# karapostK/hassaku

Measured on AMD Instinct MI355X. Metric: BPR triplets/sec, higher is better.
Workload: dtype f32

## Files before the change

### hassaku_amd/_lib.py

```python
import ctypes
import os
from ctypes import POINTER, c_char_p, c_double, c_int, c_int32, c_int64, c_uint64, c_void_p

_HERE = os.path.dirname(os.path.abspath(__file__))
LIB_PATH = os.environ.get('HSK_LIB_PATH') or os.path.join(_HERE, 'libhassaku_hip.so')

_lib = None


class HskBprmfState(ctypes.Structure):
    _fields_ = [
        ('user_emb', c_void_p), ('item_emb', c_void_p), ('item_bias', c_void_p),
        ('user_bias', c_void_p), ('global_bias', c_void_p),
        ('m_user_emb', c_void_p), ('v_user_emb', c_void_p),
        ('m_item_emb', c_void_p), ('v_item_emb', c_void_p),
        ('m_item_bias', c_void_p), ('v_item_bias', c_void_p),
        ('m_user_bias', c_void_p), ('v_user_bias', c_void_p),
        ('m_global_bias', c_void_p), ('v_global_bias', c_void_p),
        ('n_users', c_int64), ('n_items', c_int64), ('dim', c_int64),
        ('lr', c_double), ('beta1', c_double), ('beta2', c_double), ('eps', c_double), ('wd', c_double),
        ('step', c_int64),
        ('csr_indptr', c_void_p), ('csr_indices', c_void_p),
        ('coo_user', c_void_p), ('coo_item', c_void_p),
        ('nnz', c_int64),
        ('seed', c_uint64),
        ('workspace', c_void_p), ('workspace_bytes', c_int64),
        ('max_batch', c_int64), ('max_cols', c_int64),
        ('lazy_users', c_int32), ('timing_mask', c_int32),
        ('timing', c_void_p), ('aux', c_void_p),
        ('timing_every', c_int32), ('loss_kind', c_int32),
        ('opt_kind', c_int32), ('lazy_items', c_int32),
        ('ssm_log_adjust', c_double),
        ('alias_prob', c_void_p), ('alias_idx', c_void_p),
        ('graph_chunk', c_int32), ('catchup_apart', c_int32),
        ('loss_out', c_void_p), ('status', c_void_p),
        ('flush_every', c_int32), ('ws_sharded', c_int32),
        ('frozen_hyper', c_double * 5), ('frozen_opt', c_int32), ('frozen_valid', c_int32),
        ('timing_now', c_int32), ('reserved3', c_int32),
    ]


class HskBprmfShard(ctypes.Structure):
    _fields_ = [
        ('base', HskBprmfState),
        ('world', c_int32), ('rank', c_int32),
        ('n_users_global', c_int64), ('n_items_global', c_int64),
        ('item_lo', c_int64), ('capacity', c_int64), ('entry_cap', c_int64),
        ('shard_ws', c_void_p), ('shard_ws_bytes', c_int64),
        ('rows_send', c_void_p), ('rows_all', c_void_p),
        ('dU_all', c_void_p), ('grads_mine', c_void_p),
        ('s0', c_void_p), ('gsum', c_void_p),
        ('ssm_send', c_void_p), ('ssm_all', c_void_p),
        ('cur_batch', c_int64), ('cur_cols', c_int64),
        ('cur_set', c_int32), ('phase', c_int32),
    ]


SIGNATURES = {
    'hsk_version': (c_int, []),
    'hsk_last_error': (c_char_p, []),
    'hsk_device_info': (c_int, [POINTER(c_int32), POINTER(c_int32), c_char_p, c_int32]),
    'hsk_mf_scores': (c_int, [c_void_p] * 5 + [c_int64] * 3 + [c_void_p, c_void_p, c_int64, c_int64,
                                                              c_void_p, c_void_p, c_void_p]),
    'hsk_bpr_loss_grad': (c_int, [c_void_p, c_int64, c_int64, c_void_p, c_void_p, c_void_p, c_void_p]),
    'hsk_rec_loss_grad': (c_int, [c_int32, c_void_p, c_int64, c_int64, c_double, c_void_p, c_void_p, c_void_p, c_void_p]),
    'hsk_mf_backward': (c_int, [c_void_p, c_void_p, c_int64, c_int64, c_int64, c_void_p, c_void_p, c_int64,
                                c_int64, c_void_p] + [c_void_p] * 5 + [c_void_p, c_void_p]),
    'hsk_embedding_gather': (c_int, [c_void_p, c_int64, c_int64, c_void_p, c_int64, c_void_p, c_void_p, c_void_p]),
    'hsk_embedding_backward_ws_bytes': (c_int64, [c_int64, c_int64]),
    'hsk_embedding_backward': (c_int, [c_void_p, c_void_p, c_int64, c_int64, c_int64, c_void_p, c_void_p, c_int64,
                                       c_void_p, c_void_p]),
    'hsk_sparse_rows_sum': (c_int, [c_void_p, c_int64, c_int64, c_void_p, c_void_p, c_int64, c_void_p, c_int64,
                                    c_void_p, c_void_p, c_void_p]),
    'hsk_sparse_rows_offsets': (c_int, [c_void_p, c_int64, c_void_p, c_int64, c_void_p, c_void_p, c_void_p]),
    'hsk_sparse_rows_sum_backward_ws_bytes': (c_int64, [c_int64, c_int64]),
    'hsk_sparse_rows_sum_backward': (c_int, [c_void_p, c_void_p, c_void_p, c_int64, c_int64, c_void_p, c_int64,
                                             c_void_p, c_int64, c_int64, c_void_p, c_void_p, c_int64, c_void_p,
                                             c_void_p]),
    'hsk_adamw_dense': (c_int, [c_void_p] * 4 + [c_int64] + [c_double] * 5 + [c_int64, c_void_p]),
    'hsk_opt_dense': (c_int, [c_int] + [c_void_p] * 4 + [c_int64] + [c_double] * 5 + [c_int64, c_void_p]),
    'hsk_sample_negatives_uniform': (c_int, [c_void_p, c_void_p, c_int64, c_int64, c_void_p, c_int64, c_int64,
                                             c_uint64, c_uint64, c_void_p, c_void_p, c_void_p]),
    'hsk_sample_negatives_alias': (c_int, [c_void_p, c_void_p, c_int64, c_int64, c_void_p, c_void_p, c_void_p, c_int64,
                                           c_int64, c_uint64, c_uint64, c_void_p, c_void_p, c_void_p]),
    'hsk_bprmf_workspace_bytes': (c_int64, [c_int64] * 5),
    'hsk_bprmf_flush_cadence': (c_int32, [POINTER(HskBprmfState), c_int32, c_int64]),
    'hsk_shard_base_workspace_bytes': (c_int64, [c_int64] * 5),
    'hsk_synth_degrees': (c_int, [c_int64, c_int32, c_int32, c_uint64, c_void_p, c_void_p]),
    'hsk_synth_fill': (c_int, [c_int64, c_int64, c_int32, c_int32, c_uint64, c_void_p, c_void_p, c_void_p, c_void_p]),
    'hsk_bprmf_init_workspace': (c_int, [POINTER(HskBprmfState), c_void_p]),
    'hsk_bprmf_train_step': (c_int, [POINTER(HskBprmfState), c_void_p, c_void_p, c_int64, c_int64, c_void_p]),
    'hsk_bprmf_train_step_sampled': (c_int, [POINTER(HskBprmfState), c_void_p, c_int64, c_int64, c_int64,
                                             c_void_p]),
    'hsk_bprmf_train_steps': (c_int, [POINTER(HskBprmfState), c_void_p, c_int64, c_int64, c_int64, c_int64,
                                      c_void_p]),
    'hsk_bprmf_last_sort': (c_int, [POINTER(HskBprmfState), c_int64, c_void_p, c_void_p, c_void_p]),
    'hsk_key_sort_plan': (c_int, [c_int64, c_int64, c_int, POINTER(c_int64)]),
    'hsk_key_sort_ws_bytes': (c_int64, [c_int64, c_int64, c_int]),
    'hsk_key_sort': (c_int, [c_void_p, c_int64, c_int64, c_void_p, c_void_p, c_void_p, c_void_p, c_void_p, c_void_p,
                             c_int64, c_void_p, c_void_p]),
    'hsk_bprmf_graph_replays': (c_int64, [POINTER(HskBprmfState)]),
    'hsk_bprmf_batch_columns': (c_int64, [POINTER(HskBprmfState), c_int64, c_int64]),
    'hsk_eval_set_arith': (None, [c_int]),
    'hsk_timing_create': (c_void_p, []),
    'hsk_timing_destroy': (None, [c_void_p]),
    'hsk_timing_collect': (c_int, [c_void_p, POINTER(c_double), POINTER(c_int64)]),
    'hsk_aux_create': (c_void_p, []),
    'hsk_aux_destroy': (None, [c_void_p]),
    'hsk_bprmf_hint_next': (c_int, [POINTER(HskBprmfState), c_void_p, c_int64, c_int64, c_int64]),
    'hsk_bprmf_hint_after_run': (c_int, [POINTER(HskBprmfState), c_void_p, c_int64, c_int64, c_int64]),
    'hsk_bprmf_hint_after_run_n': (c_int, [POINTER(HskBprmfState), c_void_p, c_int64, c_int64, c_int64, c_int64]),
    'hsk_bprmf_pipelined_steps': (c_int64, [POINTER(HskBprmfState)]),
    'hsk_bprmf_set_pipeline': (None, [c_int]),
    'hsk_shard_workspace_bytes': (c_int64, [c_int64] * 4),
    'hsk_shard_init': (c_int, [POINTER(HskBprmfShard), c_void_p]),
    'hsk_shard_prepare': (c_int, [POINTER(HskBprmfShard), c_void_p, c_int64, c_int64, c_int64, c_int32, c_void_p]),
    'hsk_shard_discard': (c_int, [POINTER(HskBprmfShard), c_int32, c_void_p]),
    'hsk_shard_pack': (c_int, [POINTER(HskBprmfShard), c_int64, c_int64, c_int32, c_void_p]),
    'hsk_shard_pos_scores': (c_int, [POINTER(HskBprmfShard), c_void_p]),
    'hsk_shard_forward': (c_int, [POINTER(HskBprmfShard), c_void_p]),
    'hsk_shard_pos_fix': (c_int, [POINTER(HskBprmfShard), c_void_p]),
# ... 105 lines not shown
```

### hassaku_amd/csrc/hsk_fused.hip

```cpp
#include <hip/hip_ext.h>
#include "hsk_sampler.h"
#include "hsk_sort.h"
#include "hsk_step_kernels.h"
#include "hsk_item_sliced.h"
#include "hsk_fwd_small.h"
#include "hsk_fwd_part.h"
#include <stdlib.h>

#include <algorithm>
#include <utility>
#include <vector>

#ifndef HSK_FWD_R
#define HSK_FWD_R 4
#endif
#ifndef HSK_FWD_PART_R
#define HSK_FWD_PART_R 3
#endif
#define HSK_ADAM_TAB_LEN 65536
#define HSK_FLUSH_NEVER (1 << 30)

#define HSK_PART_MAX 8
#define HSK_GROUP_MAX 8
static int hsk_group_rule(int64_t n_items, int64_t dim, int64_t batch, int64_t n_cols) {
// ... 530 lines not shown
  return hsk_flush_cadence(st, table, (double)touched_rows);
}

static int hsk_launch_flush(hsk_bprmf_state* st, const hsk_ws& w, hipStream_t stream, int which = 3,
                            const int* g_poison = nullptr) {
  const int U = (int)st->n_users, D = (int)st->dim;
  if (st->step == 0) return HSK_OK;
  const hsk_adamw_consts c = hsk_make_adamw_consts(st->lr, st->beta1, st->beta2, st->eps, st->wd, st->step, st->opt_kind);
#define HSK_FLUSH(VV, GEN)                                                                                       \
  k_user_flush<VV, GEN><<<(unsigned)U, 256, 0, stream>>>(st->user_emb, st->m_user_emb, st->v_user_emb, st->user_bias, \
                                                         st->m_user_bias, st->v_user_bias, w.last_step, U, D,         \
                                                         (int)st->step, c, w.adam_tab, HSK_ADAM_TAB_LEN, g_poison)
  const bool gen = st->opt_kind != HSK_OPT_ADAMW;
  static const int wave_on = getenv("HSK_FLUSH_WAVE") ? atoi(getenv("HSK_FLUSH_WAVE")) : 1;
  const bool wave = wave_on && D <= 64 * 8 * ((D % 4 == 0) ? 4 : (D % 2 == 0) ? 2 : 1);
  auto wave_sweep = [&](float* P, float* M, float* V_, float* Pb, float* Mb, float* Vb, int* last, int n_rows) {
    return hsk_dispatch_dim(D, [&](auto v_, auto n_, auto f_) {
      constexpr int V = decltype(v_)::value, NCH = decltype(n_)::value;
      constexpr bool FULL = decltype(f_)::value;
      const unsigned grid = (unsigned)((n_rows + 3) / 4);
      if (gen)
        k_row_flush_wave<V, NCH, FULL, true><<<grid, 256, 0, stream>>>(P, M, V_, Pb, Mb, Vb, last, n_rows, D, (int)st->step, c,
                                                                     w.adam_tab, HSK_ADAM_TAB_LEN, g_poison);
      else
        k_row_flush_wave<V, NCH, FULL, false><<<grid, 256, 0, stream>>>(P, M, V_, Pb, Mb, Vb, last, n_rows, D, (int)st->step, c,
                                                                      w.adam_tab, HSK_ADAM_TAB_LEN, g_poison);
      return HSK_OK;
    });
  };
  if (wave) {
    if (st->lazy_users && (which & 1)) {
      const int rc = wave_sweep(st->user_emb, st->m_user_emb, st->v_user_emb, st->user_bias, st->m_user_bias, st->v_user_bias,
                                w.last_step, U);
      if (rc != HSK_OK) return rc;
    }
    if (st->lazy_items && (which & 2)) {
      const int rc = wave_sweep(st->item_emb, st->m_item_emb, st->v_item_emb, st->item_bias, st->m_item_bias, st->v_item_bias,
                                w.last_step_i, (int)st->n_items);
      if (rc != HSK_OK) return rc;
    }
    HSK_LAUNCH_CHECK();
    return HSK_OK;
  }
  if (st->lazy_users && (which & 1)) {
    if (D % 2 == 0) {
      if (gen) HSK_FLUSH(2, true); else HSK_FLUSH(2, false);
    } else {
      if (gen) HSK_FLUSH(1, true); else HSK_FLUSH(1, false);
    }
  }
#undef HSK_FLUSH
  if (st->lazy_items && (which & 2)) {
    const int I = (int)st->n_items;
    if (gen)
      k_user_flush<2, true><<<(unsigned)I, 256, 0, stream>>>(st->item_emb, st->m_item_emb, st->v_item_emb, st->item_bias,
                                                            st->m_item_bias, st->v_item_bias, w.last_step_i, I, D,
                                                            (int)st->step, c, w.adam_tab, HSK_ADAM_TAB_LEN, g_poison);
    else
      k_user_flush<2, false><<<(unsigned)I, 256, 0, stream>>>(st->item_emb, st->m_item_emb, st->v_item_emb, st->item_bias,
                                                             st->m_item_bias, st->v_item_bias, w.last_step_i, I, D,
                                                             (int)st->step, c, w.adam_tab, HSK_ADAM_TAB_LEN, g_poison);
  }
  HSK_LAUNCH_CHECK();
  return HSK_OK;
}

static int hsk_periodic_flush(hsk_bprmf_state* st, const hsk_ws& w, hipStream_t stream, int64_t step_before,
                              double user_rows, double entries, const int* g_poison = nullptr) {
  int which = 0;
  if (st->lazy_users) {
    const int64_t F = hsk_flush_cadence(st, 0, user_rows);
    if (st->step / F != step_before / F) which |= 1;
  }
  if (st->lazy_items) {
    const int64_t F = hsk_flush_cadence(st, 1, hsk_touched_rows((double)st->n_items, entries));
    if (st->step / F != step_before / F) which |= 2;
  }
  if (!which) return HSK_OK;
  int rc = HSK_OK;
  HSK_STAGE(HSK_STAGE_USER, rc = hsk_launch_flush(st, w, stream, which, g_poison));
  return rc;
}

template <int V, int NCH, bool FULL, int R, bool APPLY>
static void hsk_launch_item_pass(const hsk_bprmf_state* st, const hsk_ws& w, const float* Urows, const int* urow_index,
                                 int K, const hsk_adamw_consts& c, float* gI_out, float* gIb_out, hipStream_t stream,
                                 int64_t n_entries = 0, const hsk_user_lazy_args* ua = nullptr,
                                 const hsk_ahead_args* aa = nullptr, int n_part = 1, const int* g_ovf = nullptr,
                                 const int* g_poison = nullptr, const hsk_ride_item* ri = nullptr) {
  const bool part = n_part > 1;
  const int I = (int)st->n_items, D = (int)st->dim;
  if (D % 2 != 0) {
    k_item_update<V, NCH, FULL, R, APPLY><<<(unsigned)hsk_ceil_div(I, 4), 256, 0, stream>>>(
        Urows, st->item_emb, st->item_bias, st->m_item_emb, st->v_item_emb, st->m_item_bias, st->v_item_bias,
        urow_index, w.g_s, w.perm, w.offsets, I, K, D, c, gI_out, gIb_out, g_ovf, g_poison);
    return;
  }
  constexpr int VSC = (V == 4) ? 4 : 2;
  const int ipw = 1;
  const int vs = VSC;
  const int n_sl = (int)hsk_ceil_div(D, 64 * vs);
  static const int rows_on = getenv("HSK_ITEM_ROWS") ? atoi(getenv("HSK_ITEM_ROWS")) : 1;
  static const int rows_lazy = getenv("HSK_ITEM_ROWS_LAZY") ? atoi(getenv("HSK_ITEM_ROWS_LAZY")) : 1;
  const bool whole_rows = APPLY && ua && rows_on && (n_entries <= 64 * 1024 || (rows_lazy && st->lazy_items)) && !part;
  const int n_slices_pad = whole_rows ? 0 : (n_sl < 8 && 8 % n_sl == 0) ? n_sl : (int)hsk_align_up(n_sl, 8);
  const bool lazy = APPLY && st->lazy_items;
  const int64_t n_list = lazy ? std::min<int64_t>(I, n_entries) : I;
  const unsigned groups = (unsigned)hsk_align_up(hsk_ceil_div(n_list, 4 * ipw), 8);
  const hsk_item_args ia = {Urows, st->item_emb, st->item_bias, st->m_item_emb, st->v_item_emb, st->m_item_bias,
                            st->v_item_bias, urow_index, w.g_s, w.perm, w.offsets, I, K, D, n_slices_pad, ipw, c,
                            gI_out, gIb_out, w.touched, w.n_touched, w.last_step_i, (int)st->step, w.pend,
                            ua ? ua->desc : nullptr, ua ? ua->rel : 0, w.adam_tab, HSK_ADAM_TAB_LEN, n_part};
  const bool gen = APPLY && st->opt_kind != HSK_OPT_ADAMW;
  const unsigned nblk = groups * (whole_rows ? 1 : n_slices_pad);
  if (APPLY && ua) {
    const int dense = ua->n_users > 0;
    const int nub = (int)hsk_align_up(hsk_ceil_div(dense ? ua->n_users : ua->B, 4) + 1, 8);
    const hsk_ahead_args ahead = aa ? *aa : hsk_ahead_args{};
    const int item_oct = (int)(nblk / 8);
    int n_ahead_oct = ahead.coo_user ? (int)hsk_ceil_div(hsk_ceil_div(ahead.n, 4), 8) : 0;
    n_ahead_oct = std::min(n_ahead_oct, item_oct);
    const int stride = n_ahead_oct ? item_oct / n_ahead_oct : 0;
    const int nab_big = ahead.coo_user ? (int)hsk_align_up(hsk_ceil_div(ahead.n, 4), 8) : 0;

#define HSK_ITEM_USER(VS, GEN, LZ)                                                                             \
  do {                                                                                                         \
    if (whole_rows)                                                                                            \
      k_item_user_small<V, NCH, FULL, GEN, LZ><<<nblk + (unsigned)(nub + 8 * n_ahead_oct), 256, 0, stream>>>(    \
          ia, *ua, nub, dense, ahead, n_ahead_oct, stride);                                                    \
    else if (part) {                                                                                           \
      if constexpr (V == 4 && FULL && !LZ)                                                                      \
        k_item_user<V, NCH, FULL, VS, GEN, LZ, true><<<nblk + (unsigned)nub + (unsigned)(ri ? ri->n_total : 0), 256, 0, \
                                                       stream>>>(ia, *ua, nub, dense, ahead, 0,                \
                                                                 ri ? *ri : hsk_ride_item{});                  \
    } else                                                                                                     \
      k_item_user<V, NCH, FULL, VS, GEN, LZ><<<nblk + (unsigned)(nub + (LZ ? nab_big : 0)), 256, 0, stream>>>(   \
          ia, *ua, nub, dense, ahead, LZ ? nab_big : 0);                                                       \
  } while (0)
    if (gen) { if (lazy) HSK_ITEM_USER(VSC, true, true); else HSK_ITEM_USER(VSC, true, false); }
    else     { if (lazy) HSK_ITEM_USER(VSC, false, true); else HSK_ITEM_USER(VSC, false, false); }
#undef HSK_ITEM_USER
    return;
  }
  static const int rows_shard = getenv("HSK_ITEM_ROWS_SHARD") ? atoi(getenv("HSK_ITEM_ROWS_SHARD")) : 1;
  if (APPLY && !part && lazy && rows_shard) {
    const unsigned nb = (unsigned)hsk_ceil_div(n_list, 4);
    hsk_item_args ir = ia;
    ir.n_slices_pad = 0;
    if constexpr (APPLY) {
      if (gen) k_item_update_rows<V, NCH, FULL, true, true><<<nb, 256, 0, stream>>>(ir, g_ovf, g_poison);
      else     k_item_update_rows<V, NCH, FULL, false, true><<<nb, 256, 0, stream>>>(ir, g_ovf, g_poison);
    }
    return;
  }
#define HSK_ITEM_SLICED(VS, GEN, LZ)                                                   \
  do {                                                                                 \
    if (part) {                                                                        \
      if constexpr (APPLY && V == 4 && FULL && !LZ)                                    \
        k_item_update_sliced<APPLY, VS, GEN, LZ, true><<<nblk, 256, 0, stream>>>(ia, g_ovf, g_poison);   \
    } else                                                                             \
      k_item_update_sliced<APPLY, VS, GEN, LZ><<<nblk, 256, 0, stream>>>(ia, g_ovf, g_poison);          \
  } while (0)
  if (gen) { if (lazy) HSK_ITEM_SLICED(VSC, true, true); else HSK_ITEM_SLICED(VSC, true, false); }
  else     { if (lazy) HSK_ITEM_SLICED(VSC, false, true); else HSK_ITEM_SLICED(VSC, false, false); }
#undef HSK_ITEM_SLICED
}

static inline double hsk_loss_norm(int kind, double batch, double n_cols) {
  if (kind == HSK_LOSS_BCE) return 1.0 / (batch * n_cols);
  if (kind == HSK_LOSS_SSM) return 1.0 / batch;
  return 1.0 / (batch * (n_cols - 1.0));
}

static int hsk_launch_prep_sample(const hsk_bprmf_state* st, const hsk_ws& w, const int64_t* order, int64_t start,
                                  int64_t batch, int64_t n_neg, uint64_t stream_id, hipStream_t stream) {
  const hsk_aux* ax = (const hsk_aux*)st->aux;
  const hsk_step_desc* desc = ax ? ax->g_desc : nullptr;
  const int n_part = hsk_part_rule_st(st, batch, n_neg);
  HSK_STAGE(HSK_STAGE_PREP, k_prep_sample<<<(unsigned)hsk_ceil_div(batch, 4), 256, 0, stream>>>(
                                st->coo_user, st->coo_item, order, start, (int)batch, (int)n_neg, st->csr_indptr,
                                st->csr_indices, (int)st->n_items, st->seed, stream_id, w.u32, w.it32, w.owner, w.cnt,
                                st->status, 0, hsk_alias{st->alias_prob, st->alias_idx}, desc, desc ? (int)stream_id : 0,
                                w.stamp, n_part));
  HSK_LAUNCH_CHECK();
  return HSK_OK;
}

static inline bool hsk_capturing(const hsk_bprmf_state* st);

static int hsk_launch_sort(const hsk_bprmf_state* st, const hsk_ws& w, int64_t total, hipStream_t stream,
                           const int* n_dev = nullptr) {
  const int I = (int)st->n_items;
  const hsk_sort_choice sc = hsk_choose_sort(st->n_items, total, st->lazy_items != 0);
  HSK_REQUIRE(sc.kind != HSK_SORT_UNSUPPORTED, HSK_ERR_UNSUPPORTED, "item sort: n_items too large");
  int* tl = st->lazy_items ? w.touched : nullptr;
  int* tn = st->lazy_items ? w.n_touched : nullptr;
  if (sc.kind == HSK_SORT_LDS) {
    const size_t lds = sc.lds_bytes;
    if (lds > 65536 && !hsk_capturing(st))
      HSK_HIP(hipFuncSetAttribute((const void*)k_sort_lds, hipFuncAttributeMaxDynamicSharedMemorySize, (int)lds));
    HSK_STAGE(HSK_STAGE_SCATTER, (k_sort_lds<<<1, 1024, lds, stream>>>(w.it32, (int)total, I, w.perm, w.offsets, tl, tn, n_dev)));
    HSK_LAUNCH_CHECK();
    return HSK_OK;
  }
  if (sc.kind != HSK_SORT_TWO_LEVEL) {
    const int nbits = sc.nbits;
    HSK_STAGE(HSK_STAGE_SCATTER, {
// ... 1201 lines not shown
```

### hassaku_amd/csrc/hsk_item_sliced.h

```cpp
#pragma once
#include "hsk_rows.h"
#include "hsk_step_kernels.h"
#include "hsk_fwd_part.h"

#ifndef HSK_ITEM_MLP
#define HSK_ITEM_MLP 4
#endif
template <int VS>
__device__ __forceinline__ hsk_vec<VS> hsk_ldg_stream(const float* p) {
  if constexpr (hsk_stream_policy(HSK_STREAM_ITEM) == HSK_ST_NT) {
    hsk_vec<VS> r;
#pragma unroll
    for (int i = 0; i < VS; ++i) r.v[i] = __builtin_nontemporal_load(p + i);
    return r;
  } else {
    return hsk_ldg<VS>(p);
  }
}

#ifdef HSK_DEBUG_XCC
__device__ unsigned hsk_dbg_xcc[64];
#endif
struct hsk_item_args {
  const float* Uw;
// ... 59 lines not shown
  const int n_list = LAZY ? hsk_uniform_i(*n_touched) : n_items;
  for (int t = 0; t < items_per_wave; ++t) {
    const int idx = first + t;
    if (idx >= n_list) return;
    const int i = LAZY ? hsk_uniform_i(touched[idx]) : idx;
    const int beg = hsk_uniform_i(offsets[i]);
    const int end = hsk_uniform_i(offsets[i + 1]);
    hsk_vec<VS> p = hsk_zero<VS>(), m = hsk_zero<VS>(), v = hsk_zero<VS>();
    if (APPLY && live) {
      p = hsk_ldg_stream<VS>(Iw + (long long)i * D + d);
      m = hsk_ldg_stream<VS>(mI + (long long)i * D + d);
      v = hsk_ldg_stream<VS>(vI + (long long)i * D + d);
    }
    hsk_vec<VS> acc = hsk_zero<VS>();
    float gb_lane = 0.f;
    for (int c0 = beg; c0 < end; c0 += 64) {
      const int nr = min(64, end - c0);
      int myu = 0;
      float myg = 0.f;
      if (lane < nr) {
        const int e = perm[c0 + lane];
        const int bpos = e / K;
        myg = PART ? hsk_entry_weight<true>(a, e, bpos) : g_s[e];
        myu = u32 ? u32[bpos] : bpos;
      }
      gb_lane += myg;
      for (int j = 0; j < nr; j += HSK_ITEM_MLP) {
        hsk_vec<VS> val[HSK_ITEM_MLP];
#pragma unroll
        for (int r = 0; r < HSK_ITEM_MLP; ++r)
          val[r] = (j + r < nr && live) ? hsk_ldg<VS>(Uw + (long long)hsk_readlane_i(myu, min(j + r, 63)) * D + d)
                                        : hsk_zero<VS>();
#pragma unroll
        for (int r = 0; r < HSK_ITEM_MLP; ++r)
          if (j + r < nr) {
            const float g = hsk_readlane_f(myg, j + r);
#pragma unroll
            for (int q = 0; q < VS; ++q) acc.v[q] = fmaf(g, val[r].v[q], acc.v[q]);
          }
      }
    }
    if (APPLY) {
      const int behind = (LAZY && !GEN && a.pend) ? (step - 1) - hsk_uniform_i(a.pend[idx]) : 0;
      for (int r = 0; r < behind; ++r) {
#pragma unroll
        for (int q = 0; q < VS; ++q) {
          m.v[q] = fmaf(c.w1, -m.v[q], m.v[q]);
          v.v[q] = v.v[q] * c.beta2;
        }
      }
      if (live) {
#pragma unroll
        for (int q = 0; q < VS; ++q) hsk_adamw_update<GEN>(p.v[q], m.v[q], v.v[q], acc.v[q], c);
        constexpr int POL = LAZY ? HSK_ST_PLAIN : hsk_stream_policy(HSK_STREAM_ITEM);
        hsk_stg_as<POL, VS>(Iw + (long long)i * D, d, D, p);
        hsk_stg_as<POL, VS>(mI + (long long)i * D, d, D, m);
        hsk_stg_as<POL, VS>(vI + (long long)i * D, d, D, v);
      }
      if (slice == 0 && Ib) {
        const float gbias = hsk_wave_sum(gb_lane);
        if (lane == 0) {
          float pb = Ib[i], mb = mIb[i], vb = vIb[i];
          for (int r = 0; r < behind; ++r) {
            mb = fmaf(c.w1, -mb, mb);
            vb = vb * c.beta2;
          }
          hsk_adamw_update<GEN>(pb, mb, vb, gbias, c);
          Ib[i] = pb;
          mIb[i] = mb;
          vIb[i] = vb;
        }
      }
      if (LAZY && slice == 0 && lane == 0) last_step_i[i] = step;
    } else {
      if (live) hsk_stg<VS>(gI_out + (long long)i * D + d, acc);
      if (slice == 0 && gIb_out) {
        const float gbias = hsk_wave_sum(gb_lane);
        if (lane == 0) gIb_out[i] = gbias;
      }
    }
  }
}

template <int V, int NCH, bool FULL, bool GEN, bool LAZY>
__device__ __forceinline__ void hsk_item_row_body(const hsk_item_args& a, int bid) {
  const int lane = hsk_lane();
  const int idx = bid * 4 + hsk_uniform_i(threadIdx.x >> 6);
  const int n_list = LAZY ? hsk_uniform_i(*a.n_touched) : a.n_items;
  if (idx >= n_list) return;
  hsk_adamw_consts c = a.c;
  int step = a.step;
  hsk_resolve_step(a.desc, a.rel, a.ctab, a.ctab_len, step, c);
  const int i = LAZY ? hsk_uniform_i(a.touched[idx]) : idx;
  const int D = a.D, K = a.K;
  using Row = hsk_row<V, NCH>;
  const int beg = hsk_uniform_i(a.offsets[i]);
  const int end = hsk_uniform_i(a.offsets[i + 1]);
  float* prow = a.Iw + (long long)i * D;
  float* mrow = a.mI + (long long)i * D;
  float* vrow = a.vI + (long long)i * D;
  Row p, m, v, acc;
  hsk_row_load<V, NCH, FULL>(p, prow, lane, D);
  hsk_row_load<V, NCH, FULL>(m, mrow, lane, D);
  hsk_row_load<V, NCH, FULL>(v, vrow, lane, D);
  float pb = 0.f, mb = 0.f, vb = 0.f;
  if (a.Ib && lane == 0) {
    pb = a.Ib[i];
    mb = a.mIb[i];
    vb = a.vIb[i];
  }
  hsk_row_zero(acc);
  float gb_lane = 0.f;
  for (int c0 = beg; c0 < end; c0 += 64) {
    const int nr = min(64, end - c0);
    int myu = 0;
    float myg = 0.f;
    if (lane < nr) {
      const int e = a.perm[c0 + lane];
      myg = a.g_s[e];
      myu = a.u32 ? a.u32[e / K] : e / K;
    }
    gb_lane += myg;
    for (int j = 0; j < nr; j += 4) {
      Row buf[4];
#pragma unroll
      for (int r = 0; r < 4; ++r)
        if (j + r < nr) hsk_row_load<V, NCH, FULL>(buf[r], a.Uw + (long long)hsk_readlane_i(myu, min(j + r, 63)) * D, lane, D);
#pragma unroll
      for (int r = 0; r < 4; ++r)
        if (j + r < nr) hsk_row_axpy(acc, hsk_readlane_f(myg, j + r), buf[r]);
    }
  }
  const int behind = (LAZY && !GEN && a.pend) ? (step - 1) - hsk_uniform_i(a.pend[idx]) : 0;
  for (int r = 0; r < behind; ++r) {
#pragma unroll
    for (int cc = 0; cc < NCH; ++cc)
#pragma unroll
      for (int q = 0; q < V; ++q) {
        m.c[cc].v[q] = fmaf(c.w1, -m.c[cc].v[q], m.c[cc].v[q]);
        v.c[cc].v[q] = v.c[cc].v[q] * c.beta2;
      }
    mb = fmaf(c.w1, -mb, mb);
    vb = vb * c.beta2;
  }
#pragma unroll
  for (int cc = 0; cc < NCH; ++cc)
#pragma unroll
    for (int q = 0; q < V; ++q) hsk_adamw_update<GEN>(p.c[cc].v[q], m.c[cc].v[q], v.c[cc].v[q], acc.c[cc].v[q], c);
  hsk_row_store<V, NCH, FULL>(p, prow, lane, D);
  hsk_row_store<V, NCH, FULL>(m, mrow, lane, D);
  hsk_row_store<V, NCH, FULL>(v, vrow, lane, D);
  if (a.Ib) {
    const float gbias = hsk_wave_sum(gb_lane);
    if (lane == 0) {
      hsk_adamw_update<GEN>(pb, mb, vb, gbias, c);
      a.Ib[i] = pb;
      a.mIb[i] = mb;
      a.vIb[i] = vb;
    }
  }
  if (LAZY && lane == 0) a.last_step_i[i] = step;
}

template <bool APPLY, int VS, bool GEN, bool LAZY = false, bool PART = false>
__global__ __launch_bounds__(256) void k_item_update_sliced(hsk_item_args a, const int* __restrict__ g_ovf = nullptr,
                                                            const int* __restrict__ g_poison = nullptr) {
  if (APPLY && hsk_guard_skip(g_ovf, g_poison)) return;
  hsk_item_sliced_body<APPLY, VS, GEN, LAZY, PART>(a, (int)blockIdx.x);
}

template <int V, int NCH, bool FULL, bool GEN, bool LAZY>
__global__ __launch_bounds__(256) void k_item_update_rows(hsk_item_args a, const int* __restrict__ g_ovf = nullptr,
                                                          const int* __restrict__ g_poison = nullptr) {
  if (hsk_guard_skip(g_ovf, g_poison)) return;
  hsk_item_row_body<V, NCH, FULL, GEN, LAZY>(a, (int)blockIdx.x);
}

template <int V, int NCH, bool FULL, int VS, bool GEN, bool LAZYI, bool PART = false>
__global__ __launch_bounds__(256) __attribute__((amdgpu_waves_per_eu(8, 8)))
void k_item_user(hsk_item_args ia, hsk_user_lazy_args ua, int n_user_blocks, int dense_users, hsk_ahead_args aa,
                 int n_ahead_blocks, hsk_ride_item ri = hsk_ride_item{}) {
  constexpr int POL_OWNER = LAZYI ? HSK_ST_PLAIN : hsk_stream_policy(HSK_STREAM_OWNER);
  int bid = (int)blockIdx.x;
  if (PART) {
    if (bid < ri.n_total) {
      __shared__ int ride_lds[HSK_SORT_SCATTER_LDS];
      if (bid < ri.C.n_blocks) {
        hsk_sort_scatter_body(ri.C.it32, ri.C.n_entries, ri.C.plan, ri.C.hist, ri.C.btot, ri.C.perm1, ri.C.bstart, bid, ride_lds);
      } else if (bid - ri.C.n_blocks < ri.H.n_blocks) {
        hsk_sort_hist_body(ri.H.it32, ri.H.n_entries, ri.H.plan, ri.H.hist, bid - ri.C.n_blocks, ride_lds);
      }
      return;
    }
    bid -= ri.n_total;
  }
  if (bid < n_user_blocks) {
    if (dense_users)
      hsk_user_update_dense_body<V, NCH, FULL, GEN, PART, POL_OWNER>(ua, bid);
    else
      hsk_user_update_lazy_body<V, NCH, FULL, GEN, PART, POL_OWNER>(ua, bid);
    return;
  }
  if (LAZYI && bid < n_user_blocks + n_ahead_blocks) {
    hsk_user_ahead_body<V, NCH, FULL, GEN>(aa, bid - n_user_blocks);
    return;
  }
#ifdef HSK_DEBUG_XCC
  if (threadIdx.x == 0) {
    unsigned xcc;
    asm volatile("s_getreg_b32 %0, hwreg(HW_REG_XCC_ID)" : "=s"(xcc));
    atomicAdd(&hsk_dbg_xcc[((bid - n_user_blocks) & 7) * 8 + (xcc & 7)], 1u);
  }
#endif
  hsk_item_sliced_body<true, VS, GEN, LAZYI, PART>(ia, bid - n_user_blocks - (LAZYI ? n_ahead_blocks : 0));
}

template <int V, int NCH, bool FULL, bool GEN, bool LAZYI>
__global__ __launch_bounds__(256) void k_item_user_small(hsk_item_args ia, hsk_user_lazy_args ua, int n_user_blocks,
                                                         int dense_users, hsk_ahead_args aa, int n_ahead_oct,
                                                         int stride) {
  const int bid = (int)blockIdx.x;
  if (bid < n_user_blocks) {
    if (dense_users)
      hsk_user_update_dense_body<V, NCH, FULL, GEN>(ua, bid);
    else
      hsk_user_update_lazy_body<V, NCH, FULL, GEN>(ua, bid);
    return;
  }
  const int q = (bid - n_user_blocks) >> 3, r = bid & 7;
  int item_oct = q;
  if (n_ahead_oct > 0) {
    const int period = stride + 1, full = n_ahead_oct * period;
    if (q < full) {
      const int k = q / period, j = q - k * period;
      if (j == stride) {
        hsk_user_ahead_body<V, NCH, FULL, GEN>(aa, k * 8 + r);
        return;
      }
      item_oct = k * stride + j;
    } else {
      item_oct = n_ahead_oct * stride + (q - full);
    }
  }
  hsk_item_row_body<V, NCH, FULL, GEN, LAZYI>(ia, item_oct * 8 + r);
}
```

### hassaku_amd/hip_ops.py

```python
import ctypes
from typing import Optional, Sequence, Tuple

import torch

from hassaku_amd import _lib
from hassaku_amd._lib import HskBprmfState

ADAM_BETA1, ADAM_BETA2, ADAM_EPS = 0.9, 0.999, 1e-8


def _stream() -> int:
    return torch.cuda.current_stream().cuda_stream


def _p(t: Optional[torch.Tensor]) -> Optional[int]:
    return None if t is None else t.data_ptr()


def _chk(t: Optional[torch.Tensor], dtype, name: str, shape: Optional[Tuple[int, ...]] = None, optional=False):
    if t is None:
        if optional:
            return
        raise ValueError(f'{name} must not be None')
    if not t.is_cuda:
# ... 344 lines not shown
    _chk(u_idx, torch.int64, 'u_idx')
    n_users = csr_indptr.numel() - 1
    B = u_idx.numel()
    out = torch.empty((B, n_neg), dtype=torch.int64, device=u_idx.device)
    if alias is None:
        _lib.check(lib.hsk_sample_negatives_uniform(_p(csr_indptr), _p(csr_indices), n_users, n_items, _p(u_idx), B,
                                                    n_neg, seed, stream_id, _p(out), _p(status), _stream()),
                   'hsk_sample_negatives_uniform')
    else:
        prob, idx = alias
        _chk(prob, torch.float32, 'alias prob', (n_items,))
        _chk(idx, torch.int32, 'alias idx', (n_items,))
        _lib.check(lib.hsk_sample_negatives_alias(_p(csr_indptr), _p(csr_indices), n_users, n_items, _p(prob), _p(idx),
                                                  _p(u_idx), B, n_neg, seed, stream_id, _p(out), _p(status),
                                                  _stream()), 'hsk_sample_negatives_alias')
    return out


class BprMfFusedState:

    def __init__(self, user_emb, item_emb, item_bias=None, user_bias=None, global_bias=None, *, lr, wd,
                 max_batch, max_cols, beta1=ADAM_BETA1, beta2=ADAM_BETA2, eps=None, seed=0,
                 csr_indptr=None, csr_indices=None, coo_user=None, coo_item=None, lazy_users='auto', overlap=True,
                 loss='bpr', log_adjust=0.0, alias=None, optimizer='adamw', lazy_items='auto', graph_chunk=0,
                 flush_every=0):
        _lib.require_gpu()
        if optimizer not in OPT_KINDS:
            raise ValueError(f'Optimizer {optimizer} not yet implemented')
        eps = opt_eps(optimizer, eps)
        self.lib = _lib.load()
        n_users, dim = user_emb.shape
        n_items = item_emb.shape[0]
        _chk(user_emb, torch.float32, 'user_emb')
        _chk(item_emb, torch.float32, 'item_emb', (n_items, dim))
        for t, name, n in ((item_bias, 'item_bias', n_items), (user_bias, 'user_bias', n_users),
                           (global_bias, 'global_bias', 1)):
            _chk(t, torch.float32, name, optional=True)
            if t is not None and t.numel() != n:
                raise ValueError(f'{name} has {t.numel()} elements, expected {n}')
        dev = user_emb.device
        self.device = dev
        self.params = dict(user_emb=user_emb, item_emb=item_emb, item_bias=item_bias, user_bias=user_bias,
                           global_bias=global_bias)
        self.m = {k: (torch.zeros_like(t) if t is not None else None) for k, t in self.params.items()}
        self.v = {k: (torch.zeros_like(t) if t is not None else None) for k, t in self.params.items()}
        self.loss_out = torch.zeros(2, dtype=torch.float64, device=dev)
        self.status = torch.zeros(1, dtype=torch.int32, device=dev)
        self.max_batch, self.max_cols = int(max_batch), int(max_cols)
        nbytes = self.lib.hsk_bprmf_workspace_bytes(n_users, n_items, dim, self.max_batch, self.max_cols)
        if nbytes <= 0:
            raise ValueError('invalid workspace request')
        self.workspace = torch.empty(nbytes, dtype=torch.uint8, device=dev)
        self.csr_indptr, self.csr_indices, self.coo_user, self.coo_item = csr_indptr, csr_indices, coo_user, coo_item
        if csr_indptr is not None:
            _chk(csr_indptr, torch.int64, 'csr_indptr', (n_users + 1,))
            _chk(csr_indices, torch.int32, 'csr_indices')
            _chk(coo_user, torch.int32, 'coo_user')
            _chk(coo_item, torch.int32, 'coo_item', tuple(coo_user.shape))

        st = HskBprmfState()
        for k, t in self.params.items():
            setattr(st, k, _p(t))
            setattr(st, 'm_' + k, _p(self.m[k]))
            setattr(st, 'v_' + k, _p(self.v[k]))
        st.n_users, st.n_items, st.dim = n_users, n_items, dim
        st.lr, st.beta1, st.beta2, st.eps, st.wd = lr, beta1, beta2, eps, wd
        st.opt_kind = OPT_KINDS[optimizer]
        if lazy_items == 'auto':
            lazy_items = (dim % 2 == 0 and n_items >= 2 * self.max_batch * self.max_cols
                          and n_items * dim > LAZY_USERS_MIN_ELEMENTS)
        st.lazy_items = 1 if lazy_items else 0
        st.step = 0
        st.csr_indptr, st.csr_indices = _p(csr_indptr), _p(csr_indices)
        st.coo_user, st.coo_item = _p(coo_user), _p(coo_item)
        st.nnz = 0 if coo_user is None else coo_user.numel()
        st.seed = seed & 0xFFFFFFFFFFFFFFFF
        st.workspace, st.workspace_bytes = _p(self.workspace), nbytes
        st.max_batch, st.max_cols = self.max_batch, self.max_cols
        if lazy_users == 'auto':
            lazy_users = n_users > 8 * self.max_batch
        st.lazy_users = 1 if lazy_users else 0
        st.graph_chunk = int(graph_chunk)
        st.catchup_apart = 0
        st.flush_every, st.ws_sharded = int(flush_every), 0
        st.timing_mask = 0
        if loss not in LOSS_KINDS:
            raise ValueError(f'unknown loss {loss!r}')
        if loss == 'bce' and (user_bias is not None or global_bias is not None):
            raise ValueError('the fused bce step treats user/global bias as gradient-free; use the autograd path')
        st.loss_kind, st.ssm_log_adjust = LOSS_KINDS[loss], float(log_adjust)
        self.alias = alias
        if alias is not None:
            _chk(alias[0], torch.float32, 'alias prob', (n_items,))
            _chk(alias[1], torch.int32, 'alias idx', (n_items,))
        st.alias_prob, st.alias_idx = (None, None) if alias is None else (_p(alias[0]), _p(alias[1]))
        st.timing = None
        st.timing_every = 1
        self._timing = None
        self._aux = self.lib.hsk_aux_create() if overlap else None
        self._hint_order = None
        st.aux = self._aux
        st.loss_out, st.status = _p(self.loss_out), _p(self.status)
        self.st = st
        _lib.check(self.lib.hsk_bprmf_init_workspace(ctypes.byref(st), _stream()), 'hsk_bprmf_init_workspace')

    @property
    def step_count(self) -> int:
        return int(self.st.step)

    def step(self, u_idx: torch.Tensor, i_idx: torch.Tensor):
        _chk(u_idx, torch.int64, 'u_idx')
        _chk(i_idx, torch.int64, 'i_idx')
        if i_idx.dim() != 2 or u_idx.shape != (i_idx.shape[0],):
            raise ValueError(f'u_idx {tuple(u_idx.shape)} / i_idx {tuple(i_idx.shape)}: expected [B] and [B,1+N]')
        B, K = i_idx.shape
        _lib.check(self.lib.hsk_bprmf_train_step(ctypes.byref(self.st), _p(u_idx), _p(i_idx), B, K, _stream()),
                   'hsk_bprmf_train_step')

    def step_sampled(self, order: Optional[torch.Tensor], start: int, batch: int, n_neg: int):
        if order is not None:
            _chk(order, torch.int64, 'order')
            if start + batch > order.numel():
                raise ValueError('order too short')
        _lib.check(self.lib.hsk_bprmf_train_step_sampled(ctypes.byref(self.st), _p(order), start, batch, n_neg,
                                                         _stream()), 'hsk_bprmf_train_step_sampled')

    def steps_sampled(self, order: Optional[torch.Tensor], start: int, n_steps: int, batch: int, n_neg: int):
        if order is not None:
            _chk(order, torch.int64, 'order')
            if start + n_steps * batch > order.numel():
                raise ValueError('order too short')
        _lib.check(self.lib.hsk_bprmf_train_steps(ctypes.byref(self.st), _p(order), start, n_steps, batch, n_neg,
                                                  _stream()), 'hsk_bprmf_train_steps')

    def flush_cadence(self, batch: Optional[int] = None):
        import math
        b = self.max_batch if batch is None else int(batch)
        n_items = self.params['item_emb'].shape[0]
        touched = max(1, int(n_items * (1.0 - math.exp(-b * self.max_cols / n_items))))
        ref = ctypes.byref(self.st)
        return int(self.lib.hsk_bprmf_flush_cadence(ref, 0, b)), int(self.lib.hsk_bprmf_flush_cadence(ref, 1, touched))

    def graph_replays(self) -> int:
        return int(self.lib.hsk_bprmf_graph_replays(ctypes.byref(self.st)))

    def pipelined_steps(self) -> int:
        return int(self.lib.hsk_bprmf_pipelined_steps(ctypes.byref(self.st)))

    def hint_next(self, order: Optional[torch.Tensor], start: int, batch: int, n_neg: int):
        if self._aux is None:
            return
        if order is not None and batch > 0:
            _chk(order, torch.int64, 'order')
            if start + batch > order.numel():
                raise ValueError('order too short')
        self._hint_order = order
        _lib.check(self.lib.hsk_bprmf_hint_next(ctypes.byref(self.st), _p(order), start, batch, n_neg),
                   'hsk_bprmf_hint_next')

    def hint_after_run(self, order: Optional[torch.Tensor], start: int, batch: int, n_neg: int, n_batches: int = 1):
        if self._aux is None:
            return
        self._hint_order = order
        _lib.check(self.lib.hsk_bprmf_hint_after_run_n(ctypes.byref(self.st), _p(order), start, batch, n_neg,
                                                       int(n_batches)), 'hsk_bprmf_hint_after_run_n')

# ... 603 lines not shown
```

### include/hassaku_hip.h

```cpp
#ifndef HASSAKU_HIP_H
#define HASSAKU_HIP_H

#include <stdint.h>

#ifdef __cplusplus
extern "C" {
#endif

typedef void* hsk_stream_t;

enum {
  HSK_OK = 0,
  HSK_ERR_INVALID = 1,
  HSK_ERR_UNSUPPORTED = 2,
  HSK_ERR_HIP = 3
};

enum { HSK_LOSS_BPR = 0, HSK_LOSS_BCE = 1, HSK_LOSS_SSM = 2 };

enum {
  HSK_OPT_ADAMW = 0,
  HSK_OPT_ADAM = 1,
  HSK_OPT_ADAGRAD = 2
};
// ... 31 lines not shown
int hsk_embedding_gather(const float* table, int64_t n_rows, int64_t dim, const int64_t* idx, int64_t n,
                         float* out, int32_t* status, hsk_stream_t stream);
int64_t hsk_embedding_backward_ws_bytes(int64_t n_rows, int64_t n);
int hsk_embedding_backward(const float* grad_out, const int64_t* idx, int64_t n, int64_t n_rows, int64_t dim,
                           float* grad_table, void* ws, int64_t ws_bytes, int32_t* status, hsk_stream_t stream);

int hsk_sparse_rows_sum(const float* Wt, int64_t n_in, int64_t dim, const int64_t* indptr, const int32_t* indices,
                        int64_t n_rows_csr, const int64_t* idx, int64_t n, float* out, int32_t* status,
                        hsk_stream_t stream);
int hsk_sparse_rows_offsets(const int64_t* indptr, int64_t n_rows_csr, const int64_t* idx, int64_t n,
                            int64_t* pair_off, int32_t* status, hsk_stream_t stream);
int64_t hsk_sparse_rows_sum_backward_ws_bytes(int64_t n_in, int64_t n_pairs);
int hsk_sparse_rows_sum_backward(const float* g, const int64_t* indptr, const int32_t* indices, int64_t n_rows_csr,
                                 int64_t n_in, const int64_t* idx, int64_t n, const int64_t* pair_off, int64_t n_pairs,
                                 int64_t dim, float* grad_Wt, void* ws, int64_t ws_bytes, int32_t* status,
                                 hsk_stream_t stream);

int hsk_adamw_dense(float* p, const float* g, float* m, float* v, int64_t n,
                    double lr, double beta1, double beta2, double eps, double wd, int64_t step,
                    hsk_stream_t stream);

int hsk_opt_dense(int opt_kind, float* p, const float* g, float* m, float* v, int64_t n,
                  double lr, double beta1, double beta2, double eps, double wd, int64_t step,
                  hsk_stream_t stream);

int hsk_sample_negatives_uniform(const int64_t* csr_indptr, const int32_t* csr_indices,
                                 int64_t n_users, int64_t n_items,
                                 const int64_t* u_idx, int64_t batch, int64_t n_neg,
                                 uint64_t seed, uint64_t stream_id,
                                 int64_t* neg_out, int32_t* status, hsk_stream_t stream);

int hsk_sample_negatives_alias(const int64_t* csr_indptr, const int32_t* csr_indices,
                               int64_t n_users, int64_t n_items,
                               const float* alias_prob, const int32_t* alias_idx,
                               const int64_t* u_idx, int64_t batch, int64_t n_neg,
                               uint64_t seed, uint64_t stream_id,
                               int64_t* neg_out, int32_t* status, hsk_stream_t stream);


typedef struct hsk_bprmf_state {
  float* user_emb;
  float* item_emb;
  float* item_bias;
  float* user_bias;
  float* global_bias;
  float* m_user_emb;   float* v_user_emb;
  float* m_item_emb;   float* v_item_emb;
  float* m_item_bias;  float* v_item_bias;
  float* m_user_bias;  float* v_user_bias;
  float* m_global_bias; float* v_global_bias;
  int64_t n_users, n_items, dim;
  double lr, beta1, beta2, eps, wd;
  int64_t step;
  const int64_t* csr_indptr;
  const int32_t* csr_indices;
  const int32_t* coo_user;
  const int32_t* coo_item;
  int64_t nnz;
  uint64_t seed;
  void* workspace;
  int64_t workspace_bytes;
  int64_t max_batch, max_cols;
  int32_t lazy_users;
  int32_t timing_mask;
  void* timing;
  void* aux;
  int32_t timing_every;
  int32_t loss_kind;
  int32_t opt_kind;
  int32_t lazy_items;
  double ssm_log_adjust;
  const float* alias_prob;
  const int32_t* alias_idx;
  int32_t graph_chunk;
  int32_t catchup_apart;
  double* loss_out;
  int32_t* status;
  int32_t flush_every;
  int32_t ws_sharded;
  double frozen_hyper[5];
  int32_t frozen_opt;
  int32_t frozen_valid;
  int32_t timing_now;
  int32_t reserved3;
} hsk_bprmf_state;

int64_t hsk_bprmf_workspace_bytes(int64_t n_users, int64_t n_items, int64_t dim,
                                  int64_t max_batch, int64_t max_cols);
int32_t hsk_bprmf_flush_cadence(const hsk_bprmf_state* st, int32_t table, int64_t touched_rows);
int hsk_bprmf_init_workspace(hsk_bprmf_state* st, hsk_stream_t stream);

int hsk_bprmf_train_step(hsk_bprmf_state* st, const int64_t* u_idx, const int64_t* i_idx,
                         int64_t batch, int64_t n_cols, hsk_stream_t stream);

int hsk_bprmf_train_step_sampled(hsk_bprmf_state* st, const int64_t* order, int64_t start,
                                 int64_t batch, int64_t n_neg, hsk_stream_t stream);

enum {
  HSK_STAGE_PREP = 0,
  HSK_STAGE_SCAN = 1,
  HSK_STAGE_SCATTER = 2,
  HSK_STAGE_FWD = 3,
  HSK_STAGE_ITEM = 4,
  HSK_STAGE_USER = 5,
  HSK_STAGE_FINISH = 6,
  HSK_STAGE_COUNT = 7
};

void* hsk_timing_create(void);
void hsk_timing_destroy(void* timing);
int hsk_timing_collect(void* timing, double* ms_sum, int64_t* count);

void* hsk_aux_create(void);
void hsk_aux_destroy(void* aux);

int hsk_bprmf_hint_next(hsk_bprmf_state* st, const int64_t* order, int64_t start, int64_t batch, int64_t n_neg);

int hsk_bprmf_train_steps(hsk_bprmf_state* st, const int64_t* order, int64_t start, int64_t n_steps, int64_t batch,
                          int64_t n_neg, hsk_stream_t stream);

int hsk_bprmf_hint_after_run(hsk_bprmf_state* st, const int64_t* order, int64_t start, int64_t batch, int64_t n_neg);
int hsk_bprmf_hint_after_run_n(hsk_bprmf_state* st, const int64_t* order, int64_t start, int64_t batch, int64_t n_neg,
                               int64_t n_batches);

int64_t hsk_bprmf_graph_replays(const hsk_bprmf_state* st);
int64_t hsk_bprmf_pipelined_steps(const hsk_bprmf_state* st);
void hsk_bprmf_set_pipeline(int on);

int hsk_bprmf_flush(hsk_bprmf_state* st, hsk_stream_t stream);

int hsk_bprmf_last_batch(const hsk_bprmf_state* st, int64_t batch, int64_t n_cols,
                         int64_t* u_out, int64_t* i_out, hsk_stream_t stream);

void hsk_eval_set_arith(int form);

int64_t hsk_bprmf_batch_columns(const hsk_bprmf_state* st, int64_t batch, int64_t n_cols);

int hsk_bprmf_last_sort(const hsk_bprmf_state* st, int64_t n_entries, int32_t* perm_out, int32_t* offsets_out,
                        hsk_stream_t stream);

int hsk_key_sort_plan(int64_t n_keys, int64_t n_entries, int want_touched, int64_t out[8]);
int64_t hsk_key_sort_ws_bytes(int64_t n_keys, int64_t n, int want_touched);
int hsk_key_sort(const int64_t* keys, int64_t n, int64_t n_keys, const int32_t* n_dev, int32_t* perm, int32_t* offsets,
                 int32_t* touched, int32_t* n_touched, void* ws, int64_t ws_bytes, int32_t* status, hsk_stream_t stream);

enum { HSK_STATUS_SHARD_OVERFLOW = 4 };

typedef struct hsk_bprmf_shard {
  hsk_bprmf_state base;
  int32_t world, rank;
  int64_t n_users_global, n_items_global;
  int64_t item_lo;
  int64_t capacity;
  int64_t entry_cap;
  void* shard_ws;
  int64_t shard_ws_bytes;
  float* rows_send;
  float* rows_all;
  float* dU_all;
  float* grads_mine;
  float* s0;
  float* gsum;
  float* ssm_send;
  float* ssm_all;
  int64_t cur_batch, cur_cols;
  int32_t cur_set;
  int32_t phase;
// ... 184 lines not shown
```

Before: 2.519 billion.

## Add paired-row item update kernel using half-wave gathers and permlane32 swaps

Adds a new item-update path for eager AdamW with no urow index and no whole-row mode. Each wave covers 128-float slices, and its two half-waves fetch different user rows in one vector load, then exchange halves with permlane32_swap. The path turns on by a heuristic when the gathered user working set is larger than a hot-bytes threshold and each item has many entries on average. It can also be forced through a new state field or an environment variable. The aim is better coalescing and more loads in flight for the gather-accumulate, at the cost of extra cross-lane swaps and added selection logic.

```diff
diff --git a/hassaku_amd/_lib.py b/hassaku_amd/_lib.py
--- a/hassaku_amd/_lib.py
+++ b/hassaku_amd/_lib.py
@@ -36,7 +36,7 @@
         ('loss_out', c_void_p), ('status', c_void_p),
         ('flush_every', c_int32), ('ws_sharded', c_int32),
         ('frozen_hyper', c_double * 5), ('frozen_opt', c_int32), ('frozen_valid', c_int32),
-        ('timing_now', c_int32), ('reserved3', c_int32),
+        ('timing_now', c_int32), ('item_pair', c_int32),
     ]
 
 
diff --git a/hassaku_amd/csrc/hsk_fused.hip b/hassaku_amd/csrc/hsk_fused.hip
--- a/hassaku_amd/csrc/hsk_fused.hip
+++ b/hassaku_amd/csrc/hsk_fused.hip
@@ -636,6 +636,9 @@
   return rc;
 }
 
+#ifndef HSK_ITEM_PAIR_HOT_BYTES
+#define HSK_ITEM_PAIR_HOT_BYTES (2 << 20)
+#endif
 template <int V, int NCH, bool FULL, int R, bool APPLY>
 static void hsk_launch_item_pass(const hsk_bprmf_state* st, const hsk_ws& w, const float* Urows, const int* urow_index,
                                  int K, const hsk_adamw_consts& c, float* gI_out, float* gIb_out, hipStream_t stream,
@@ -653,19 +656,28 @@
   constexpr int VSC = (V == 4) ? 4 : 2;
   const int ipw = 1;
   const int vs = VSC;
-  const int n_sl = (int)hsk_ceil_div(D, 64 * vs);
+  int n_sl = (int)hsk_ceil_div(D, 64 * vs);
   static const int rows_on = getenv("HSK_ITEM_ROWS") ? atoi(getenv("HSK_ITEM_ROWS")) : 1;
   static const int rows_lazy = getenv("HSK_ITEM_ROWS_LAZY") ? atoi(getenv("HSK_ITEM_ROWS_LAZY")) : 1;
   const bool whole_rows = APPLY && ua && rows_on && (n_entries <= 64 * 1024 || (rows_lazy && st->lazy_items)) && !part;
+  const bool lazy = APPLY && st->lazy_items;
+  const bool gen = APPLY && st->opt_kind != HSK_OPT_ADAMW;
+  static const int pair_env = getenv("HSK_ITEM_PAIR") ? atoi(getenv("HSK_ITEM_PAIR")) : -1;
+  bool pair = false;
+  if (APPLY && V == 4 && (FULL || !part) && ua && !urow_index && (int64_t)ua->B * D < (1 << 30) && !whole_rows &&
+      !lazy && !gen) {
+    const int64_t hot = (int64_t)ua->B * std::min(D, 256) * 4;
+    pair = st->item_pair ? st->item_pair > 0 : pair_env >= 0 ? pair_env != 0
+                                                              : hot > HSK_ITEM_PAIR_HOT_BYTES && n_entries >= 8 * (int64_t)I;
+  }
+  if (pair) n_sl = (int)hsk_ceil_div(D, 128);
   const int n_slices_pad = whole_rows ? 0 : (n_sl < 8 && 8 % n_sl == 0) ? n_sl : (int)hsk_align_up(n_sl, 8);
-  const bool lazy = APPLY && st->lazy_items;
   const int64_t n_list = lazy ? std::min<int64_t>(I, n_entries) : I;
   const unsigned groups = (unsigned)hsk_align_up(hsk_ceil_div(n_list, 4 * ipw), 8);
   const hsk_item_args ia = {Urows, st->item_emb, st->item_bias, st->m_item_emb, st->v_item_emb, st->m_item_bias,
                             st->v_item_bias, urow_index, w.g_s, w.perm, w.offsets, I, K, D, n_slices_pad, ipw, c,
                             gI_out, gIb_out, w.touched, w.n_touched, w.last_step_i, (int)st->step, w.pend,
                             ua ? ua->desc : nullptr, ua ? ua->rel : 0, w.adam_tab, HSK_ADAM_TAB_LEN, n_part};
-  const bool gen = APPLY && st->opt_kind != HSK_OPT_ADAMW;
   const unsigned nblk = groups * (whole_rows ? 1 : n_slices_pad);
   if (APPLY && ua) {
     const int dense = ua->n_users > 0;
@@ -677,6 +689,18 @@
     const int stride = n_ahead_oct ? item_oct / n_ahead_oct : 0;
     const int nab_big = ahead.coo_user ? (int)hsk_align_up(hsk_ceil_div(ahead.n, 4), 8) : 0;
 
+    if (pair) {
+      if constexpr (APPLY && V == 4) {
+        if (part) {
+          if constexpr (FULL)
+            k_item_user_pair<NCH, FULL, true><<<nblk + (unsigned)nub + (unsigned)(ri ? ri->n_total : 0), 256, 0, stream>>>(
+                ia, *ua, nub, dense, ri ? *ri : hsk_ride_item{});
+        } else {
+          k_item_user_pair<NCH, FULL><<<nblk + (unsigned)nub, 256, 0, stream>>>(ia, *ua, nub, dense);
+        }
+      }
+      return;
+    }
 #define HSK_ITEM_USER(VS, GEN, LZ)                                                                             \
   do {                                                                                                         \
     if (whole_rows)                                                                                            \
diff --git a/hassaku_amd/csrc/hsk_item_sliced.h b/hassaku_amd/csrc/hsk_item_sliced.h
--- a/hassaku_amd/csrc/hsk_item_sliced.h
+++ b/hassaku_amd/csrc/hsk_item_sliced.h
@@ -165,6 +165,136 @@
   }
 }
 
+#ifndef HSK_ITEM_PAIR_MLP
+#define HSK_ITEM_PAIR_MLP 4
+#endif
+
+__device__ __forceinline__ void hsk_half_swap(float& a, float& b) {
+  const auto r = __builtin_amdgcn_permlane32_swap(__float_as_uint(a), __float_as_uint(b), false, false);
+  a = __uint_as_float(r[0]);
+  b = __uint_as_float(r[1]);
+}
+__device__ __forceinline__ void hsk_pair_swap(hsk_vec<4>& x) {
+  hsk_half_swap(x.v[0], x.v[2]);
+  hsk_half_swap(x.v[1], x.v[3]);
+}
+
+template <int MLP, bool TAIL>
+__device__ __forceinline__ void hsk_pair_gather(const float* __restrict__ Uw, int D, unsigned hm, unsigned dl, int myu,
+                                                float myg, int j, int nr, hsk_vec<2>& acc) {
+  hsk_vec<4> val[MLP];
+#pragma unroll
+  for (int r = 0; r < MLP; ++r) {
+    const int e0 = j + 2 * r;
+    const unsigned r0 = (unsigned)hsk_readlane_i(myu, TAIL ? min(e0, 63) : e0) * (unsigned)D;
+    const unsigned r1 = (unsigned)hsk_readlane_i(myu, TAIL ? min(e0 + 1, 63) : e0 + 1) * (unsigned)D;
+    val[r] = hsk_ldg<4>(Uw + (((r0 & ~hm) | (r1 & hm)) + dl));
+  }
+#pragma unroll
+  for (int r = 0; r < MLP; ++r) {
+    const int e0 = j + 2 * r;
+    hsk_pair_swap(val[r]);
+    if (!TAIL || e0 < nr) {
+      const float g0 = hsk_readlane_f(myg, e0);
+      acc.v[0] = fmaf(g0, val[r].v[0], acc.v[0]);
+      acc.v[1] = fmaf(g0, val[r].v[1], acc.v[1]);
+    }
+    if (!TAIL || e0 + 1 < nr) {
+      const float g1 = hsk_readlane_f(myg, e0 + 1);
+      acc.v[0] = fmaf(g1, val[r].v[2], acc.v[0]);
+      acc.v[1] = fmaf(g1, val[r].v[3], acc.v[1]);
+    }
+  }
+}
+
+template <bool PART>
+__device__ __forceinline__ void hsk_item_pair_body(const hsk_item_args& a, int bid) {
+  const float* __restrict__ Uw = a.Uw;
+  float* __restrict__ Iw = a.Iw;
+  float* __restrict__ Ib = a.Ib;
+  float* __restrict__ mI = a.mI;
+  float* __restrict__ vI = a.vI;
+  float* __restrict__ mIb = a.mIb;
+  float* __restrict__ vIb = a.vIb;
+  const float* __restrict__ g_s = a.g_s;
+  const int* __restrict__ perm = a.perm;
+  const int* __restrict__ offsets = a.offsets;
+  const int n_items = a.n_items, K = a.K, D = a.D, n_slices_pad = a.n_slices_pad, items_per_wave = a.items_per_wave;
+  hsk_adamw_consts c = a.c;
+  int step = a.step;
+  hsk_resolve_step(a.desc, a.rel, a.ctab, a.ctab_len, step, c);
+  const int lane = hsk_lane();
+  const int wave = hsk_uniform_i(threadIdx.x >> 6);
+  int slice, group;
+  if (n_slices_pad < 8) {
+    const int xcd = bid & 7, r = bid >> 3;
+    slice = xcd % n_slices_pad;
+    group = r * (8 / n_slices_pad) + xcd / n_slices_pad;
+  } else {
+    slice = bid % n_slices_pad;
+    group = bid / n_slices_pad;
+  }
+  constexpr int SW = 128;
+  constexpr int MLP = HSK_ITEM_PAIR_MLP;
+  const int h = lane >> 5;
+  const int d4 = slice * SW + (lane & 31) * 4;
+  const int d2 = d4 + 2 * h;
+  const bool live = d4 < D;
+  const unsigned dl = live ? (unsigned)d4 : 0u;
+  const unsigned hm = h ? ~0u : 0u;
+  if (slice * SW >= D) return;
+  const int first = (group * 4 + wave) * items_per_wave;
+  for (int t = 0; t < items_per_wave; ++t) {
+    const int i = first + t;
+    if (i >= n_items) return;
+    const int beg = hsk_uniform_i(offsets[i]);
+    const int end = hsk_uniform_i(offsets[i + 1]);
+    float* const prow = Iw + (long long)i * D;
+    float* const mrow = mI + (long long)i * D;
+    float* const vrow = vI + (long long)i * D;
+    hsk_vec<2> p = hsk_zero<2>(), m = hsk_zero<2>(), v = hsk_zero<2>();
+    if (live) {
+      p = hsk_ldg_stream<2>(prow + d2);
+      m = hsk_ldg_stream<2>(mrow + d2);
+      v = hsk_ldg_stream<2>(vrow + d2);
+    }
+    hsk_vec<2> acc = hsk_zero<2>();
+    float gb_lane = 0.f;
+    for (int c0 = beg; c0 < end; c0 += 64) {
+      const int nr = min(64, end - c0);
+      int myu = 0;
+      float myg = 0.f;
+      if (lane < nr) {
+        const int e = perm[c0 + lane];
+        const int bpos = e / K;
+        myg = PART ? hsk_entry_weight<true>(a, e, bpos) : g_s[e];
+        myu = bpos;
+      }
+      gb_lane += myg;
+      int j = 0;
+      for (; j + 2 * MLP <= nr; j += 2 * MLP) hsk_pair_gather<MLP, false>(Uw, D, hm, dl, myu, myg, j, nr, acc);
+      if (j < nr) hsk_pair_gather<MLP, true>(Uw, D, hm, dl, myu, myg, j, nr, acc);
+    }
+    if (live) {
+#pragma unroll
+      for (int q = 0; q < 2; ++q) hsk_adamw_update<false>(p.v[q], m.v[q], v.v[q], acc.v[q], c);
+      hsk_stg<2>(prow + d2, p);
+      hsk_stg<2>(mrow + d2, m);
+      hsk_stg<2>(vrow + d2, v);
+    }
+    if (slice == 0 && Ib) {
+      const float gbias = hsk_wave_sum(gb_lane);
+      if (lane == 0) {
+        float pb = Ib[i], mb = mIb[i], vb = vIb[i];
+        hsk_adamw_update<false>(pb, mb, vb, gbias, c);
+        Ib[i] = pb;
+        mIb[i] = mb;
+        vIb[i] = vb;
+      }
+    }
+  }
+}
+
 template <int V, int NCH, bool FULL, bool GEN, bool LAZY>
 __device__ __forceinline__ void hsk_item_row_body(const hsk_item_args& a, int bid) {
   const int lane = hsk_lane();
@@ -298,6 +428,33 @@
   hsk_item_sliced_body<true, VS, GEN, LAZYI, PART>(ia, bid - n_user_blocks - (LAZYI ? n_ahead_blocks : 0));
 }
 
+template <int NCH, bool FULL, bool PART = false>
+__global__ __launch_bounds__(256) __attribute__((amdgpu_waves_per_eu(8, 8)))
+void k_item_user_pair(hsk_item_args ia, hsk_user_lazy_args ua, int n_user_blocks, int dense_users, hsk_ride_item ri = hsk_ride_item{}) {
+  constexpr int POL_OWNER = hsk_stream_policy(HSK_STREAM_OWNER);
+  int bid = (int)blockIdx.x;
+  if (PART) {
+    if (bid < ri.n_total) {
+      __shared__ int ride_lds[HSK_SORT_SCATTER_LDS];
+      if (bid < ri.C.n_blocks) {
+        hsk_sort_scatter_body(ri.C.it32, ri.C.n_entries, ri.C.plan, ri.C.hist, ri.C.btot, ri.C.perm1, ri.C.bstart, bid, ride_lds);
+      } else if (bid - ri.C.n_blocks < ri.H.n_blocks) {
+        hsk_sort_hist_body(ri.H.it32, ri.H.n_entries, ri.H.plan, ri.H.hist, bid - ri.C.n_blocks, ride_lds);
+      }
+      return;
+    }
+    bid -= ri.n_total;
+  }
+  if (bid < n_user_blocks) {
+    if (dense_users)
+      hsk_user_update_dense_body<4, NCH, FULL, false, PART, POL_OWNER>(ua, bid);
+    else
+      hsk_user_update_lazy_body<4, NCH, FULL, false, PART, POL_OWNER>(ua, bid);
+    return;
+  }
+  hsk_item_pair_body<PART>(ia, bid - n_user_blocks);
+}
+
 template <int V, int NCH, bool FULL, bool GEN, bool LAZYI>
 __global__ __launch_bounds__(256) void k_item_user_small(hsk_item_args ia, hsk_user_lazy_args ua, int n_user_blocks,
                                                          int dense_users, hsk_ahead_args aa, int n_ahead_oct,
diff --git a/hassaku_amd/hip_ops.py b/hassaku_amd/hip_ops.py
--- a/hassaku_amd/hip_ops.py
+++ b/hassaku_amd/hip_ops.py
@@ -450,6 +450,7 @@
         st.lazy_users = 1 if lazy_users else 0
         st.graph_chunk = int(graph_chunk)
         st.catchup_apart = 0
+        st.item_pair = 0
         st.flush_every, st.ws_sharded = int(flush_every), 0
         st.timing_mask = 0
         if loss not in LOSS_KINDS:
diff --git a/include/hassaku_hip.h b/include/hassaku_hip.h
--- a/include/hassaku_hip.h
+++ b/include/hassaku_hip.h
@@ -137,7 +137,7 @@
   int32_t frozen_opt;
   int32_t frozen_valid;
   int32_t timing_now;
-  int32_t reserved3;
+  int32_t item_pair;
 } hsk_bprmf_state;
 
 int64_t hsk_bprmf_workspace_bytes(int64_t n_users, int64_t n_items, int64_t dim,
```

Result: faster. 2.595 billion, median of 6 (+3.0%).
